# IvanBanny/para-ortho-pca-bo

Measured on AMD Instinct MI355X. Metric: BO iterations/sec (incl. GP refit + EI opt), BBOB f15 d=40, higher is better.
Workload: dtype f64; 1 GPU; configs[1]: PCA_BO on BBOB f15 d=40, budget=450, n_DoE=120, EI, var_threshold=0.95; one run per GPU (run list f15/d40/instances 0..N-1 partitioned by pcabo.sharding), timed steps spread evenly over the 330 BO iterations of the run; num_restarts=10, raw_samples=512, batch_limit=5, maxiter=200, parallelism=run-parallel x1

## Files before the change

### para-ortho-pca-bo_amd/csrc/ctx_layout.h

```cpp
#pragma once
#include <stddef.h>

#define PCABO_BS 64
#define PCABO_SLAB 16
#define PCABO_MAXD 128
#define PCABO_PSTRIDE (2 + 2 * PCABO_MAXD)
#define PCABO_QA_MAX 416
#define PCABO_CNT_DONE 0x3fff
#define PCABO_QFLAG_WORDS 32
#define PCABO_GROUP_CNT_OFFSET 8192
#define PCABO_HYP_INV_LS 0
#define PCABO_HYP_NOISE 1
#define PCABO_HYP_MEAN_C 2
#define PCABO_HYP_ARD_FOLD 3
#define PCABO_HYP_WORDS 4
#define PCABO_OPT_REC_BASE 64
#define PCABO_OPT_REC_STRIDE 8
static_assert(PCABO_QFLAG_WORDS <= PCABO_OPT_REC_BASE, "the values of a call's restarts end in front of the records");
#define PCABO_XQ_TAIL 8
#define EXT_XN 0
#define EXT_YS PCABO_MAXD
#define EXT_HDR_RUNG (PCABO_MAXD + 1)
#define EXT_HDR_INFO (PCABO_MAXD + 2)
#define EXT_HDR 2
#define EXT_INFO_SKIP (-1)
// ... 109 lines not shown
static inline Use xq_ext_rows(const CtxShape& s, int k) { return {0, (size_t)ext_rows_cap(s, k) * k}; }
static inline Use xq_ext_vals(const CtxShape& s, int k) { return {xq_ext_rows(s, k).count, (size_t)ext_rows_cap(s, k)}; }

static inline Use partial_ext_scratch(const CtxShape& s) { return {0, 3 * (size_t)s.NPcap + EXT_SMALL}; }
struct ExtScratch {
  double *ks, *v, *w, *small;
  ExtScratch(double* partial, const CtxShape& s) : ks(partial), v(partial + s.NPcap), w(partial + 2 * (size_t)s.NPcap), small(partial + 3 * (size_t)s.NPcap) {}
};
static inline Use partial_loo(int n) { return {0, 4 * (size_t)n}; }
static inline size_t partial_loo_part(int n, int v) { return (size_t)v * n; }
static inline Use partial_post_records(int q, int NP) { return {0, (size_t)q * (NP / 64) * PCABO_PSTRIDE}; }
static inline Use partial_post_result(int q, int NP) { return {partial_post_records(q, NP).count, 3 * (size_t)q}; }

static inline Use counters_queries(int q) { return {0, (size_t)q}; }
static inline Use counters_group() { return {PCABO_GROUP_CNT_OFFSET, PCABO_QFLAG_WORDS}; }

static inline Use gram_rt(int NP, int ld) { return {0, (size_t)NP * ld}; }

static inline Use mll_partials(int NP, int M) { const size_t nb = NP / PCABO_BS; return {0, (1 + (size_t)M) * (nb * (nb + 1) / 2)}; }
static inline Use mll_result(int NP, int M) { return {mll_partials(NP, M).count, 5 + (size_t)M}; }
static inline Use hmll_result(int M) { return {0, 5 + (size_t)M}; }

static inline int opt_groups(int num_restarts, int batch_limit) { return (num_restarts + batch_limit - 1) / batch_limit; }
static inline Use xq_opt_points(int num_restarts, int kmax) { return {0, (size_t)(num_restarts + 2) * kmax}; }
static inline Use grad_opt_cands(int num_restarts, int kmax) { return {0, (size_t)num_restarts * kmax}; }
static inline Use val_opt_values(int num_restarts) { return {0, (size_t)num_restarts}; }
static inline Use val_opt_records(int ngroups) { return {PCABO_OPT_REC_BASE, (size_t)PCABO_OPT_REC_STRIDE * ngroups}; }
static inline size_t val_opt_record(int gi) { return PCABO_OPT_REC_BASE + (size_t)PCABO_OPT_REC_STRIDE * gi; }
static inline bool opt_fits(const CtxLayout& L, int num_restarts, int ngroups, int kmax) {
  return fits(val_opt_records(ngroups), L.dev[D_VAL]) && fits(xq_opt_points(num_restarts, kmax), xq_queries(L.s));
// ... 2 lines not shown
```

### para-ortho-pca-bo_amd/csrc/host_selftest.cpp

```cpp
#include "../../include/pcabo.h"
#include "host_side.h"
#include "lb_plan.h"
#include "ctx_layout.h"
#include "model_state.h"

#include <atomic>
#include <cmath>
#include <cstdint>
#include <cstdio>
#include <cstdlib>
#include <cstring>
#include <vector>

namespace {

int g_fail = 0;
#define CHECK(c, ...) do { if (!(c)) { std::fprintf(stderr, "FAIL %s:%d: ", __FILE__, __LINE__); std::fprintf(stderr, __VA_ARGS__); std::fprintf(stderr, "\n"); ++g_fail; } } while (0)

struct Lcg {
  uint64_t s;
  explicit Lcg(uint64_t seed) : s(seed * 6364136223846793005ull + 1442695040888963407ull) {}
  double uni() { s = s * 6364136223846793005ull + 1442695040888963407ull; return (double)(s >> 11) * (1.0 / 9007199254740992.0); }
};

// ... 921 lines not shown
             val_opt_record(0) == 64 && val_opt_record(ngroups - 1) + 8 == rec.start + rec.count, "the device optimiser's values and records");
    }
    for (int M : {1, s.KPcap}) {
      const Use part = mll_partials(s.NPcap, M), res = mll_result(s.NPcap, M);
      LCHECK(fits(part, L.dev[D_MLL]) && fits(res, L.dev[D_MLL]) && apart(part, res) && fits(hmll_result(M), L.host[H_MLL]) &&
             hmll_result(M).count == res.count, "the fit's results");
    }
    const Use w = small_wpca(s), x = small_imap_x(s), nb = small_norm_bounds(s);
    const PcaParts pp = pca_parts(s);
    LCHECK(fits(w, small) && fits(x, small) && fits(nb, small) && apart(w, x) && apart(w, nb) && apart(x, nb), "the three tenants of hSmall");
    LCHECK(x.count >= (size_t)max_d && nb.count >= 2 * (size_t)max_d && pca_copy_count(s, max_d, max_d) == w.count && w.count == L.dev[D_PCAOUT].count &&
           pp.data_mean + max_d <= pp.pca_mean && pp.pca_mean + max_d <= pp.evr && pp.evr + max_d <= pp.comps, "the wPCA result block");
    LCHECK(in_pack(max_n, max_d, true, true, true).total == L.dev[D_IN].count && L.dev[D_IN].count == L.host[H_IN].count, "the packed inputs");
    LCHECK(fits(counters_queries(max_q), L.dev[D_COUNTERS]) && fits(counters_group(), L.dev[D_COUNTERS]) &&
           apart(counters_queries(PCABO_QFLAG_WORDS), counters_group()), "the tickets");
    LCHECK(fits(gram_rt(s.NPcap, s.NPcap), L.dev[D_GRAM]), "the transposed root inverse");
#undef LCHECK
  }
}

struct MS {
  int n, n_base, d, k, KP, NP; double ls, s2; int kernel; double rung;
  bool have_wpca, unc; int wn, wd; bool pending, have_gp, zn, rt; int cnt_S; bool dirty; int gcur, vprev_d;
};
void expect_state(const ModelState& s, const MS& e, const char* what) {
  CHECK(s.n == e.n && s.n_base == e.n_base && s.d == e.d && s.k == e.k && s.KP == e.KP && s.NP == e.NP,
        "%s: shape n %d n_base %d d %d k %d KP %d NP %d", what, s.n, s.n_base, s.d, s.k, s.KP, s.NP);
  CHECK(s.lengthscale == e.ls && s.noise == e.s2 && s.kernel == e.kernel && s.rung == e.rung,
        "%s: hyperparameters %g %g %d rung %g", what, s.lengthscale, s.noise, s.kernel, s.rung);
  CHECK(s.have_wpca == e.have_wpca && s.wpca_uncollected == e.unc && s.wpca_n == e.wn && s.wpca_d == e.wd,
// ... 207 lines not shown
```

### para-ortho-pca-bo_amd/csrc/kernels_acq.hip

```cpp
#include "pcabo_internal.h"
#include "acq_math.h"
#include <algorithm>
#include <cstdlib>
#include <mutex>

#define PSTRIDE PCABO_PSTRIDE

#ifdef PCABO_ACQ_TIMING
__device__ unsigned long long g_acq_stamps[16];
#define STAMP(i) do { if (blockIdx.x == gridDim.x / 2 && blockIdx.y == 0 && threadIdx.x == 0) g_acq_stamps[i] = wall_clock64(); } while (0)
#define STAMP_FIN(i) do { if (blockIdx.y == 0 && threadIdx.x == 0) g_acq_stamps[i] = wall_clock64(); } while (0)
extern "C" int pcabo_debug_acq_stamps(unsigned long long* out16) {
  return hipMemcpyFromSymbol(out16, HIP_SYMBOL(g_acq_stamps), sizeof(g_acq_stamps)) == hipSuccess ? 0 : -3;
}
#else
#define STAMP(i)
#define STAMP_FIN(i)
#endif

__device__ inline void st_wt(double* p, double v) {
  __hip_atomic_store(p, v, __ATOMIC_RELAXED, __HIP_MEMORY_SCOPE_AGENT);
}

template <int SLAB>
// ... 1119 lines not shown
  const int tid = threadIdx.x, l = tid & 63, w = tid >> 6;
  const int j = blockIdx.x * 256 + tid, q0 = blockIdx.y * SC_QB;
  double ks[SC_QB];
  score_ks_block(Xq, q_total, n, k, NP, ld, ZnT, bounds4, prm, KS, ks);
  const double aj = j < n ? alpha[j] : 0.0;
#pragma unroll
  for (int q = 0; q < SC_QB; ++q) {
    const double m = wave_sum(aj * ks[q]);
    if (l == 0) s_mu[w][q] = m;
  }
  __syncthreads();
  if (tid < SC_QB && q0 + tid < q_total)
    partial[((size_t)(q0 + tid) * S + blockIdx.x) * PSTRIDE + 1] = ((s_mu[0][tid] + s_mu[1][tid]) + s_mu[2][tid]) + s_mu[3][tid];
}

template <bool STORE_V>
__global__ __launch_bounds__(256) void k_score_gemm(const double* __restrict__ R, const double* __restrict__ KS,
                                                    int q_total, int NP, int ld, int njb, double* __restrict__ partial,
                                                    double* __restrict__ V, size_t zs, size_t vzs) {
  ZRUN(R); ZRUN(KS); ZRUN(partial);
  __shared__ __attribute__((aligned(16))) double s_a[64 * PCABO_TLD];
  __shared__ __attribute__((aligned(16))) double s_b[64 * PCABO_TLD];
  __shared__ double s_red[4][64];
  const int tid = threadIdx.x, w = tid >> 6, l = tid & 63;
  const int I = blockIdx.x, qb = blockIdx.y, S = gridDim.x;
  const double* Rrow = R + (size_t)(I * 64) * ld;
  const double* Krow = KS + (size_t)(qb * 64) * ld;
  double4_t acc[4];
  tile_product_f64<false>(s_a, s_b, I + 1, [&](int J, int r, int c, double& a, double& b) {
    a = Rrow[(size_t)r * ld + J * 64 + c];
    b = (qb * 64 + r < q_total) ? Krow[(size_t)r * ld + J * 64 + c] : 0.0;
  }, acc);
  if (STORE_V) {
    V = zrun(V, vzs, blockIdx.z);
#pragma unroll
    for (int t = 0; t < 4; ++t) {
      const int a = qb * 64 + 16 * t + (l & 15);
#pragma unroll
      for (int r = 0; r < 4; ++r)
        if (a < q_total) V[(size_t)(I * 64 + 16 * w + (l >> 4) + 4 * r) * q_total + a] = acc[t][r];
    }
  }
#pragma unroll
  for (int t = 0; t < 4; ++t) {
    double v = ((acc[t][0] * acc[t][0] + acc[t][1] * acc[t][1]) + acc[t][2] * acc[t][2]) + acc[t][3] * acc[t][3];
    v += __shfl_xor(v, 16, 64);
    v += __shfl_xor(v, 32, 64);
    if (l < 16) s_red[w][16 * t + l] = v;
  }
  __syncthreads();
  if (tid < 64 && qb * 64 + tid < q_total) {
    double* rec = partial + ((size_t)(qb * 64 + tid) * S + I) * PSTRIDE;
    rec[0] = ((s_red[0][tid] + s_red[1][tid]) + s_red[2][tid]) + s_red[3][tid];
    if (I >= njb) rec[1] = 0.0;
  }
}

void launch_score_gemm(hipStream_t st, const GpModel& m, int q, const double* KS, double* partial, size_t zs, int B, double* V,
                       size_t vzs) {
  const dim3 grid(m.NP / 64, (q + 63) / 64, B);
  const int njb = (m.NP + 255) / 256;
  if (V) hipLaunchKernelGGL(k_score_gemm<true>, grid, dim3(256), 0, st, m.R, KS, q, m.NP, m.ld, njb, partial, V, zs, vzs);
  else hipLaunchKernelGGL(k_score_gemm<false>, grid, dim3(256), 0, st, m.R, KS, q, m.NP, m.ld, njb, partial, V, zs, vzs);
}

bool score_gemm_possible(int q) { return q >= 64; }

__global__ __launch_bounds__(256) void k_score_ks_only(const double* __restrict__ Xq, int q_total, int n, int k, int NP, int ld,
                                                       const double* __restrict__ ZnT, const double* __restrict__ bounds4,
                                                       AcqParams prm, double* __restrict__ KS) {
  double ks[SC_QB];
  score_ks_block(Xq, q_total, n, k, NP, ld, ZnT, bounds4, prm, KS, ks);
}

__global__ __launch_bounds__(256) void k_score_mu(const double* __restrict__ KS, int q_total, int n, int ld,
                                                  const double* __restrict__ alpha, double* __restrict__ partial, int S) {
  __shared__ double s_mu[4][SC_QB];
  const int tid = threadIdx.x, l = tid & 63, w = tid >> 6;
  const int j = blockIdx.x * 256 + tid, q0 = blockIdx.y * SC_QB;
  const double aj = j < n ? alpha[j] : 0.0;
#pragma unroll
  for (int q = 0; q < SC_QB; ++q) {
    const double ks = (j < n && q0 + q < q_total) ? KS[(size_t)(q0 + q) * ld + j] : 0.0;
    const double m = wave_sum(aj * ks);
    if (l == 0) s_mu[w][q] = m;
  }
  __syncthreads();
  if (tid < SC_QB && q0 + tid < q_total)
    partial[((size_t)(q0 + tid) * S + blockIdx.x) * PSTRIDE + 1] = ((s_mu[0][tid] + s_mu[1][tid]) + s_mu[2][tid]) + s_mu[3][tid];
}

void launch_score_ks_only(hipStream_t st, const double* Xq, int q, const GpModel& m, AcqParams p, double* KS) {
  const int njb = (m.NP + 255) / 256;
  hipLaunchKernelGGL(k_score_ks_only, dim3(njb, (q + SC_QB - 1) / SC_QB, 1), dim3(256), 0, st, Xq, q, m.n, m.k, m.NP, m.ld, m.ZnT,
                     m.bounds4, p, KS);
}
void launch_score_tail(hipStream_t st, int q, const GpModel& m, AcqParams p, const double* KS, double* partial, double* val) {
  const int S = m.NP / 64, njb = (m.NP + 255) / 256;
  hipLaunchKernelGGL(k_score_mu, dim3(njb, (q + SC_QB - 1) / SC_QB, 1), dim3(256), 0, st, KS, q, m.n, m.ld, m.alpha, partial, S);
  launch_score_gemm(st, m, q, KS, partial);
  p.want_grad = 0;
  hipLaunchKernelGGL(k_acq_combine, dim3((q + 3) / 4, 1, 1), dim3(256), 0, st, partial, q, S, m.k, m.bounds4, m.ystats, p, val,
                     (double*)nullptr, AcqBatch());
}

void launch_score_ks(hipStream_t st, const double* Xq, int q, const GpModel& m, AcqParams p, double* KS, double* partial, AcqBatch ab,
                     int B) {
  const int S = m.NP / 64, njb = (m.NP + 255) / 256;
  hipLaunchKernelGGL(k_score_ks, dim3(njb, (q + SC_QB - 1) / SC_QB, B), dim3(256), 0, st, Xq, q, m.n, m.k, m.NP, m.ld, m.ZnT, m.alpha,
                     m.bounds4, p, KS, partial, S, ab);
}

void launch_score(hipStream_t st, const double* Xq, int q, const GpModel& m, AcqParams p, double* KS, double* partial, double* val,
                  AcqBatch ab, int B) {
  const int S = m.NP / 64;
  launch_score_ks(st, Xq, q, m, p, KS, partial, ab, B);
  launch_score_gemm(st, m, q, KS, partial, ab.zs, B);
  p.want_grad = 0;
// ... 105 lines not shown
```

### para-ortho-pca-bo_amd/csrc/kernels_gp.hip

```cpp
#include "pcabo_internal.h"
#include <mutex>
#include <cstdlib>

#define BS PCABO_BS
#define TLD PCABO_TLD

__global__ __launch_bounds__(256) void k_gram(const double* __restrict__ AT, const double* __restrict__ nrm, int n,
                                              int KP, int ld, double noise, int kernel, double* __restrict__ K,
                                              const int* __restrict__ k_dev, double* __restrict__ K2,
                                              int* __restrict__ info_reset, size_t zs, const double* __restrict__ hyp) {
  const XcdTile xt_ = xcd_tile();
  ZRUNX(AT); ZRUNX(nrm); ZRUNX(K); ZRUNX(k_dev); ZRUNX(K2); ZRUNX(info_reset); ZRUNX(hyp);
  if (hyp) noise = hyp[PCABO_HYP_NOISE];
  const int ti = (int)xt_.x, tj = (int)xt_.y;
  if (info_reset && ti == 0 && tj == 0 && threadIdx.x == 0) *info_reset = 0;
  if (tj > ti) return;
  if (k_dev) KP = (*k_dev + 3) & ~3;
  const int w = threadIdx.x >> 6, l = threadIdx.x & 63;
  const int i0 = ti * BS + 16 * w, j0 = tj * BS;
  double4_t acc[4];
  for (int t = 0; t < 4; ++t) acc[t] = (double4_t){0.0, 0.0, 0.0, 0.0};
  for (int kk = 0; kk < KP; kk += 4) {
    const double* row = AT + (size_t)(kk + (l >> 4)) * ld;
    double a = row[i0 + (l & 15)];
// ... 249 lines not shown
    __syncthreads();
    double4_t x = {0.0, 0.0, 0.0, 0.0};
    for (int kk = 0; kk < BS; kk += 4) {
      double a = s_t[(16 * w + (l & 15)) * TLD + kk + (l >> 4)];
      double b = s_xk[(kk + (l >> 4)) * 16 + (l & 15)];
      x = __builtin_amdgcn_mfma_f64_16x16x4f64(a, b, x, 0, 0, 0);
    }
    for (int r = 0; r < 4; ++r)
      R[(size_t)(I * BS + 16 * w + (l >> 4) + 4 * r) * ld + c0 + (l & 15)] = x[r];
    __threadfence_block();
  }
}

__device__ __forceinline__ void rmatvec_run(const double* __restrict__ R, const double* __restrict__ y, int n, int ld,
                                            double* __restrict__ t) {
  const int w = threadIdx.x >> 6, l = threadIdx.x & 63;
  for (int rr = 0; rr < 4; ++rr) {
    const int i = blockIdx.x * 16 + w * 4 + rr;
    double s = 0.0;
    if (i < n)
      for (int j = l; j <= i; j += 64) s += R[(size_t)i * ld + j] * y[j];
    s = wave_sum(s);
    if (l == 0) t[i] = (i < n) ? s : 0.0;
  }
}
__global__ __launch_bounds__(256) void k_rmatvec(const double* __restrict__ R, const double* __restrict__ y, int n,
                                                 int ld, double* __restrict__ t, size_t zs) {
  ZRUN(R); ZRUN(y); ZRUN(t);
  rmatvec_run(R, y, n, ld, t);
}
__global__ __launch_bounds__(256) void k_rmatvec_gated(const double* __restrict__ R, const double* __restrict__ y, int n, int ld,
                                                       double* __restrict__ t, size_t zs, const int* __restrict__ gate) {
  if (*zrun(gate, zs, blockIdx.z) != 0) return;
  ZRUN(R); ZRUN(y); ZRUN(t);
  rmatvec_run(R, y, n, ld, t);
}

#define RTM_WAVES 16
__device__ __forceinline__ void rtmatvec_run(const double* __restrict__ R, const double* __restrict__ t, int n, int ld,
// ... 19 lines not shown
    out[j] = (j < n) ? s : 0.0;
  }
}
__global__ __launch_bounds__(64 * RTM_WAVES) void k_rtmatvec(const double* __restrict__ R, const double* __restrict__ t,
                                                             int n, int ld, double* __restrict__ out, size_t zs) {
  ZRUN(R); ZRUN(t); ZRUN(out);
  rtmatvec_run(R, t, n, ld, out);
}
__global__ __launch_bounds__(64 * RTM_WAVES) void k_rtmatvec_gated(const double* __restrict__ R, const double* __restrict__ t, int n,
                                                                   int ld, double* __restrict__ out, size_t zs,
                                                                   const int* __restrict__ gate) {
  if (*zrun(gate, zs, blockIdx.z) != 0) return;
  ZRUN(R); ZRUN(t); ZRUN(out);
  rtmatvec_run(R, t, n, ld, out);
}

void launch_gram(hipStream_t s, const double* AT, const double* nrm, int n, int NP, int KP, int ld, double noise,
                 int kernel, double* K, const int* k_dev, double* K2, int* info_reset, ZB zb) {
  int nb = NP / BS;
  hipLaunchKernelGGL(k_gram, dim3(nb, nb, zb.B), dim3(256), 0, s, AT, nrm, n, KP, ld, noise, kernel, K, k_dev, K2, info_reset,
                     zb.zs, zb.hyp);
}
void launch_add_jitter(hipStream_t s, double* K, int n, int ld, double jitter) {
  hipLaunchKernelGGL(k_add_jitter, dim3((n + 255) / 256), dim3(256), 0, s, K, n, ld, jitter);
}
bool chol_step_form(int NP, ZB zb) { return zb.B * (NP / BS) <= 256; }
int launch_cholesky(hipStream_t s, double* L, int NP, int ld, int* info, double* diag_scratch, ZB zb, double* R_folded) {
  const int nblk = NP / BS;
  if (chol_step_form(NP, zb)) return launch_chol_steps(s, L, NP, ld, info, diag_scratch, zb, R_folded);
  if (R_folded) return -1;
// ... 36 lines not shown
      }
    }
  }
  return 0;
}
void launch_trinv(hipStream_t s, const double* L, int NP, int ld, double* R, ZB zb) {
  const int nblk = NP / BS;
  launch_trinv_diag_w(s, L, nblk, ld, R, zb);
  hipLaunchKernelGGL(k_trinv_cols, dim3(NP / 16, 1, zb.B), dim3(256), 0, s, L, nblk, ld, R, zb.zs);
}
void launch_alpha(hipStream_t s, const double* R, const double* ys, int n, int NP, int ld, double* tmp, double* alpha,
                  ZB zb) {
  hipLaunchKernelGGL(k_rmatvec, dim3(NP / 16, 1, zb.B), dim3(256), 0, s, R, ys, n, ld, tmp, zb.zs);
  hipLaunchKernelGGL(k_rtmatvec, dim3(NP / 64, 1, zb.B), dim3(64 * RTM_WAVES), 0, s, R, tmp, n, ld, alpha, zb.zs);
}
void launch_alpha_gated(hipStream_t s, const double* R, const double* ys, int n, int NP, int ld, double* tmp, double* alpha, ZB zb,
                        const int* gate) {
  hipLaunchKernelGGL(k_rmatvec_gated, dim3(NP / 16, 1, zb.B), dim3(256), 0, s, R, ys, n, ld, tmp, zb.zs, gate);
  hipLaunchKernelGGL(k_rtmatvec_gated, dim3(NP / 64, 1, zb.B), dim3(64 * RTM_WAVES), 0, s, R, tmp, n, ld, alpha, zb.zs, gate);
}
```

### para-ortho-pca-bo_amd/csrc/kernels_gpw.hip

```cpp
#include "pcabo_internal.h"
#include <mutex>

#define BS PCABO_BS
#ifdef PCABO_ACQ_TIMING
__device__ unsigned long long g_panel_stamps[16];
extern "C" int pcabo_debug_panel_stamps(unsigned long long* out16) {
  return hipMemcpyFromSymbol(out16, HIP_SYMBOL(g_panel_stamps), sizeof(g_panel_stamps)) == hipSuccess ? 0 : -3;
}
#define PSTAMP(i) do { if (blockIdx.x == 0 && blockIdx.z == 0 && threadIdx.x == 0) g_panel_stamps[i] = wall_clock64(); } while (0)
#else
#define PSTAMP(i)
#endif
#define WLD 65

__device__ inline double lane_get(double v, int lane) {
  return __hiloint2double(__builtin_amdgcn_readlane(__double2hiint(v), lane),
                          __builtin_amdgcn_readlane(__double2loint(v), lane));
}


#define PANEL_LDS_SYNC() asm volatile("s_waitcnt lgkmcnt(0)" ::: "memory")
template <int JB, bool LOWER>
__device__ inline void tiles_colblock_to_lds(const double4_t (&acc)[4][4], double* s_t, int l) {
#pragma unroll
// ... 534 lines not shown
  InvChunk<0, 0, 0>::run(x, lb, s_lt, s_rd, xm);
  double* dst = R + (size_t)(b * BS) * ld + b * BS;
#pragma unroll
  for (int r = 0; r < BS; ++r) dst[(size_t)r * ld + c] = (r >= c) ? x[r] : 0.0;
}


void launch_chol_panel(hipStream_t s, double* L, int p, int nblocks, int ld, int* info, double* diag_scratch, ZB zb) {
  hipLaunchKernelGGL(k_chol_panel_m, dim3(nblocks, 1, zb.B), dim3(128), 0, s, L, p, ld, info, diag_scratch, zb.zs);
}
__global__ __launch_bounds__(256) void k_trinv_rowblock(const double* L, int I, int ld, double* R) {
  __shared__ __attribute__((aligned(16))) double s_t[BS * SLD];
  __shared__ __attribute__((aligned(16))) double s_xk[BS * 16];
  trinv_rowblock_chunk(L, R, I, 16 * blockIdx.x, ld, s_t, s_xk);
}
void launch_trinv_drain(hipStream_t s, const double* L, int NP, int ld, double* R) {
  const int nblk = NP / BS;
  if (nblk >= 2) hipLaunchKernelGGL(k_trinv_rowblock, dim3(4 * (nblk - 1)), dim3(256), 0, s, L, nblk - 1, ld, R);
}
int launch_chol_steps(hipStream_t s, double* L, int NP, int ld, int* info, double* diag_scratch, ZB zb, double* R) {
  static std::mutex attr_mu;
  static bool attr_done[64] = {false};
  int dev = 0;
  if (hipGetDevice(&dev) != hipSuccess || dev < 0 || dev >= 64) return -1;
  {
    std::lock_guard<std::mutex> lk(attr_mu);
    if (!attr_done[dev]) {
      if (hipFuncSetAttribute((const void*)k_chol_step, hipFuncAttributeMaxDynamicSharedMemorySize, (int)CHOL_STEP_LDS) != hipSuccess) return -1;
      attr_done[dev] = true;
    }
  }
  const int nblk = NP / BS;
  for (int J = 0; J < nblk; ++J) {
// ... 9 lines not shown
```

### para-ortho-pca-bo_amd/csrc/pcabo_api.hip

```cpp
#include "../../include/pcabo.h"
#include "pcabo_internal.h"
#include "lbfgsb.h"
#include "host_side.h"
#include "model_state.h"

#include <algorithm>
#include <atomic>
#include <chrono>
#include <thread>
#include <condition_variable>
#include <functional>
#include <mutex>
#include <cstdlib>
#include <cmath>
#include <cstdio>
#include <cstring>
#include <new>
#include <optional>
#include <vector>
#include <dirent.h>
#include <fcntl.h>
#include <signal.h>
#include <stdint.h>
#include <cerrno>
// ... 355 lines not shown
  int n, k, KP; const int* k_dev;
  double inv_ls, noise, mean_c; int kernel;
  ZB zb;
  hipEvent_t ev[2];
  bool reset_tickets;
  const double* ard_ls = nullptr;
  hipEvent_t ev_zn = nullptr;
};
template <class Phase>
static int enqueue_factor(pcabo_ctx* ctx, hipStream_t s, int n, int NP, ZB zb, Phase&& phase) {
  if (const int rc = phase(2)) return rc;
  const bool fold = !ctx->in_batch && ctx->opt_hidden_tail && zb.zs == 0 && zb.B == 1 && chol_step_form(NP, zb);
  if (launch_cholesky(s, ctx->dL, NP, ctx->ld, ctx->dInfo, ctx->dDiag, zb, fold ? ctx->dR : nullptr) != 0)
    return set_err(ctx, PCABO_ERR_HIP, "the Cholesky launches could not be set up (device or kernel attribute)%s", "");
  if (const int rc = phase(3)) return rc;
  if (fold) launch_trinv_drain(s, ctx->dL, NP, ctx->ld, ctx->dR);
  else launch_trinv(s, ctx->dL, NP, ctx->ld, ctx->dR, zb);
  launch_alpha(s, ctx->dR, ctx->dYs, n, NP, ctx->ld, ctx->dTmp, ctx->dAlpha, zb);
  if (const int rc = phase(4)) return rc;
  if (zb.zs) HIPCHK(hipMemcpy2DAsync((void*)&ctx->hm->chol_info, zb.hzs, ctx->dInfo, zb.zs, sizeof(int), zb.B, hipMemcpyDeviceToHost, s));
  else HIPCHK(hipMemcpyAsync((void*)&ctx->hm->chol_info, ctx->dInfo, sizeof(int), hipMemcpyDeviceToHost, s));
  return PCABO_OK;
}
template <class Phase>
static int enqueue_rows_dh(pcabo_ctx* ctx, hipStream_t s, const RowsDH& a, Phase&& phase) {
  const int NP = round_up(a.n, PCABO_BS);
  if (a.reset_tickets) {
    if (a.zb.zs) HIPCHK(hipMemset2DAsync(ctx->dCounters, a.zb.zs, 0, ticket_bytes(ctx), a.zb.B, s));
    else HIPCHK(hipMemsetAsync(ctx->dCounters, 0, ticket_bytes(ctx), s));
  }
// ... 469 lines not shown
    launch_acq(s, qa, xdev, nq, gp_model(ctx), p, ctx->dPartial, ctx->dCounters, ctx->dVal, ctx->dGrad, small ? ctx->hVal : nullptr,
               small ? ctx->hGrad : nullptr, small ? ctx->hm : nullptr, seq);
  }
  if (!small) {
    HIPCHK(hipMemcpyAsync(ctx->hVal, ctx->dVal, (size_t)nq * sizeof(double), hipMemcpyDeviceToHost, s));
    if (p.want_grad) HIPCHK(hipMemcpyAsync(ctx->hGrad, ctx->dGrad, (size_t)nq * k * sizeof(double), hipMemcpyDeviceToHost, s));
    HIPCHK(wait_stream(s));
    HIPCHK(hipGetLastError());
    return PCABO_OK;
  }
  return acq_published(ctx, wait_flags(ctx->hm, 0, nq, seq, deadline_in(20), &s));
}

static int score_tail(pcabo_ctx* ctx, int nq, AcqParams& p) {
  hipStream_t s = ctx->stream;
  launch_score_tail(s, nq, gp_model(ctx), p, ctx->dKS, ctx->dPartial, ctx->dVal);
  HIPCHK(hipMemcpyAsync(ctx->hVal, ctx->dVal, (size_t)nq * sizeof(double), hipMemcpyDeviceToHost, s));
  HIPCHK(wait_stream(s));
  HIPCHK(hipGetLastError());
  return PCABO_OK;
}

struct GroupLaunches {
  int g0[8], gn[8], ng = 0;
  void add(int q0, int n) { g0[ng] = q0; gn[ng] = n; ++ng; }
};
static int eval_staged_groups(pcabo_ctx* ctx, const GroupLaunches& t, AcqParams& p) {
  hipStream_t s = ctx->stream;
  const unsigned long long seq = ++ctx->seq;
  const int *g0 = t.g0, *gn = t.gn, ng = t.ng;
  QueryArgs tab;
  unsigned* ent = reinterpret_cast<unsigned*>(tab.x);
// ... 2019 lines not shown
```

### para-ortho-pca-bo_amd/csrc/pcabo_internal.h

```cpp
#pragma once
#include <hip/hip_runtime.h>
#include <stdint.h>
#include <type_traits>
#include "ctx_layout.h"

#define PCABO_TLD 66
#define PCABO_INLAUNCH_MAXQ 32
static_assert(PCABO_INLAUNCH_MAXQ == PCABO_QFLAG_WORDS, "one sequence word of the host mirror per query finished inside a launch");

typedef double double4_t __attribute__((ext_vector_type(4)));
struct QueryArgs { double x[PCABO_QA_MAX]; };
struct alignas(16) MailPair { double v; unsigned long long tag; };
static inline __host__ __device__ unsigned long long mail_mix(unsigned long long vbits) {
  const unsigned int lo = (unsigned int)vbits, hi = (unsigned int)(vbits >> 32);
  return (unsigned long long)((lo ^ hi ^ (hi >> 11)) & 0xFFFFFFu);
}
#define PCABO_MAIL_PAIRS (1 + PCABO_QA_MAX + PCABO_INLAUNCH_MAXQ + 1)
#define PCABO_SERVER_TIMEOUT_TICKS 200000000ull

#ifdef __HIPCC__
__device__ inline double fast_rcp(double x) {
  double r = __builtin_amdgcn_rcp(x);
  r = fma(fma(-x, r, 1.0), r, r);
  r = fma(fma(-x, r, 1.0), r, r);
// ... 98 lines not shown
__device__ inline double row_sum16(double v) {
  v += dpp_get<0xB1, 0xf>(v);
  v += dpp_get<0x4E, 0xf>(v);
  v += dpp_get<0x141, 0xf>(v);
  v += dpp_get<0x140, 0xf>(v);
  return v;
}
__device__ inline double wave_sum(double v) {
  v = row_sum16(v);
  v += dpp_get<0x142, 0xa>(v);
  v += dpp_get<0x143, 0xc>(v);
  return __hiloint2double(__builtin_amdgcn_readlane(__double2hiint(v), 63),
                          __builtin_amdgcn_readlane(__double2loint(v), 63));
}

template <bool KMAJOR, typename Elem>
__device__ __forceinline__ void tile_product_f64(double* s_a, double* s_b, int steps, Elem elem, double4_t (&acc)[4]) {
  const int tid = threadIdx.x, w = tid >> 6, l = tid & 63;
  double pa[16], pb[16];
  auto fetch = [&](int J) {
#pragma unroll
    for (int u = 0; u < 16; ++u) {
      const int idx = tid + 256 * u;
      elem(J, idx >> 6, idx & 63, pa[u], pb[u]);
    }
  };
  auto put = [&]() {
#pragma unroll
    for (int u = 0; u < 16; ++u) {
      const int idx = tid + 256 * u, r = idx >> 6, c = idx & 63;
      s_a[r * PCABO_TLD + c] = pa[u];
      s_b[r * PCABO_TLD + c] = pb[u];
    }
  };
#pragma unroll
  for (int t = 0; t < 4; ++t) acc[t] = (double4_t){0.0, 0.0, 0.0, 0.0};
  fetch(0);
  for (int J = 0; J < steps; ++J) {
    __syncthreads();
    put();
    if (J + 1 < steps) fetch(J + 1);
    __syncthreads();
    for (int kk = 0; kk < 64; kk += 4) {
      const double a = KMAJOR ? s_a[(kk + (l >> 4)) * PCABO_TLD + 16 * w + (l & 15)]
                              : s_a[(16 * w + (l & 15)) * PCABO_TLD + kk + (l >> 4)];
#pragma unroll
      for (int t = 0; t < 4; ++t) {
        const double b = KMAJOR ? s_b[(kk + (l >> 4)) * PCABO_TLD + 16 * t + (l & 15)]
                                : s_b[(16 * t + (l & 15)) * PCABO_TLD + kk + (l >> 4)];
        acc[t] = __builtin_amdgcn_mfma_f64_16x16x4f64(a, b, acc[t], 0, 0, 0);
      }
    }
  }
}

template <int T>
__device__ inline double lane_xor(double v) {
  if (T == 0) return dpp_get<0xB1, 0xf>(v);
  if (T == 1) return dpp_get<0x4E, 0xf>(v);
  if (T == 2) return dpp_get<0x141, 0xf>(dpp_get<0x1B, 0xf>(v));
  return dpp_get<0x128, 0xf>(v);
}
// ... 82 lines not shown
                    const double* comps, const int* k_dev, int n, int d, double* Z, ZB zb = ZB());
void launch_zstats(hipStream_t s, const double* Z, const double* y, int n, int k, const double* user_norm_bounds,
                   double* bounds4 , double* zn_mean, double* ystats,
                   double* ys, HostMirror* hm, const int* k_dev = nullptr, ZB zb = ZB(),
                   double mean_c = 0.0,
                   const double* ard_ls = nullptr);
void launch_znorm(hipStream_t s, const double* Z, int n, int k, int NP, int KP, int ld, const double* bounds4,
                  const double* zn_mean, double inv_ls, double* ZnT, double* AT, double* nrm,
                  const int* k_dev = nullptr, ZB zb = ZB());
void launch_gram(hipStream_t s, const double* AT, const double* nrm, int n, int NP, int KP, int ld, double noise,
                 int kernel, double* K, const int* k_dev = nullptr, double* K2 = nullptr, int* info_reset = nullptr,
                 ZB zb = ZB());
void launch_add_jitter(hipStream_t s, double* K, int n, int ld, double jitter);
int launch_cholesky(hipStream_t s, double* L, int NP, int ld, int* info, double* diag_scratch, ZB zb = ZB(), double* R_folded = nullptr);
bool chol_step_form(int NP, ZB zb);
void launch_trinv_drain(hipStream_t s, const double* L, int NP, int ld, double* R);
void launch_trinv(hipStream_t s, const double* L, int NP, int ld, double* R, ZB zb = ZB());
void launch_chol_panel(hipStream_t s, double* L, int p, int nblocks, int ld, int* info, double* diag_scratch, ZB zb = ZB());
int launch_chol_steps(hipStream_t s, double* L, int NP, int ld, int* info, double* diag_scratch , ZB zb = ZB(),
                      double* R = nullptr);
void launch_trinv_diag_w(hipStream_t s, const double* L, int nblk, int ld, double* R, ZB zb = ZB());
void launch_alpha(hipStream_t s, const double* R, const double* ys, int n, int NP, int ld, double* tmp, double* alpha,
                  ZB zb = ZB());
void launch_alpha_gated(hipStream_t s, const double* R, const double* ys, int n, int NP, int ld, double* tmp, double* alpha, ZB zb,
                        const int* gate);
void launch_mll_grad(hipStream_t s, bool ard, const double* R, const double* AT, const double* nrm, const double* alpha,
                     const double* L, const double* ys, int n, int NP, int KP, int ld, double* partial, double* out,
                     const int* k_dev = nullptr, ZB zb = ZB());
void launch_acq(hipStream_t s, const QueryArgs* qa, const double* Xq, int q, const GpModel& m, AcqParams p, double* partial,
                unsigned int* counters, double* val, double* grad, double* host_val, double* host_grad, HostMirror* hm,
                unsigned long long seq,
                MailPair* dev_mail = nullptr, MailPair* part_pairs = nullptr,
                AcqBatch ab = AcqBatch(), int B = 1, int table_entries = 0);
#define PCABO_GROUP_Q 5
bool acq_group_possible(int NP, int k);
int launch_acq_group(hipStream_t st, const QueryArgs* tab, int entries, const double* Xq, const GpModel& m, AcqParams p,
                     double* partial, unsigned int* counters, double* val, double* grad, double* host_val, double* host_grad,
                     HostMirror* hm, unsigned long long seq, AcqBatch ab);
// ... 9 lines not shown
                      double* KS, double* partial, double* post, double* V, double* cov, AcqBatch ab = AcqBatch(),
                      size_t vzs = 0, int B = 1);
void launch_post_chol_prep(hipStream_t st, const double* cov, int q, const double* ystats, double jitter, double* F, int* info,
                           size_t zs = 0, size_t vzs = 0, size_t szs = 0, int B = 1);
void launch_post_sample(hipStream_t st, const double* F, int q, const double* base, int S, const double* mean ,
                        double* out, size_t zs = 0, size_t szs = 0, int B = 1);
void launch_loo(hipStream_t st, const double* R, const double* alpha, const double* ys, const double* ystats, int n, int ld,
                double* out, size_t zs = 0, int B = 1);
struct GpArrays { const double* zn_mean; double *L, *R, *ZnT, *AT, *nrm, *ys; };
void launch_ext_ks(hipStream_t st, const double* X, int xi, const double* Y, int yi, const GpModel& m, double inv_ls, int kernel,
                   const ExtScratch& e, AcqBatch ab = AcqBatch(), int B = 1);
void launch_ext_append(hipStream_t st, const GpModel& m, const ExtScratch& e, int idx, int believer, double s2, double inv_ls,
                       const GpArrays& a, AcqBatch ab = AcqBatch(), int B = 1);
void launch_ext_truncate(hipStream_t st, const ExtScratch& e, int n0, int k, int NP, int ld, const GpArrays& a,
                         AcqBatch ab = AcqBatch(), int B = 1);
void launch_score_tail(hipStream_t st, int q, const GpModel& m, AcqParams p, const double* KS, double* partial, double* val);
bool acq_server_possible(int q, int n, int k, int NP);
int acq_slabs(int NP);
void launch_inverse_map(hipStream_t s, const double* z, const double* comps, const double* data_mean,
                        const double* pca_mean, int k, int d, double* x, const int* k_dev = nullptr, ZB zb = ZB(),
                        double* host_x = nullptr, HostMirror* hm = nullptr, unsigned long long seq = 0);
void launch_rt_build(hipStream_t s, const double* R, int n, int NP, int ld, double* RT, ZB zb = ZB());
bool lbfgsb_device_possible(int NP, int kmax, int batch_limit);
int launch_lbfgsb_group(hipStream_t st, const unsigned* table, int entries, int mode, int num_restarts, int maxiter, const GpModel& m,
                        const double* Xq, const double* RT, const double* bestf, const int* k_dev, double inv_ls,
                        int maximize, int acq, int kernel, double* out_x, double* out_v, size_t zs,
                        const double* hyp = nullptr,
                        int batch_limit = PCABO_GROUP_Q);
```

Baseline: 420.1 BO iterations/s.

## Fuse score tail kernels with ticketed finish and merge alpha solve into trinv drain

The scoring tail's three launches (mu, GEMM column norms, combine) become one kernel. Its blocks do either the GEMM slab or the mu block, and the last block per query group, found through an atomic ticket counter, runs the EI finish and writes values straight to host memory, so the separate device-to-host copy goes away. In the GP refit, the R*y matvec rides along in the trinv drain launch, and a tail kernel finishes the last rows, does the transposed matvec and publishes chol_info to the host mirror. This cuts launches and a memcpy per call, at the cost of a narrower GEMM tile, counter-based cross-block sync and extra correctness risk.

```diff
diff --git a/para-ortho-pca-bo_amd/csrc/ctx_layout.h b/para-ortho-pca-bo_amd/csrc/ctx_layout.h
--- a/para-ortho-pca-bo_amd/csrc/ctx_layout.h
+++ b/para-ortho-pca-bo_amd/csrc/ctx_layout.h
@@ -9,6 +9,7 @@
 #define PCABO_CNT_DONE 0x3fff
 #define PCABO_QFLAG_WORDS 32
 #define PCABO_GROUP_CNT_OFFSET 8192
+#define PCABO_SCORE_CNT_OFFSET 12288
 #define PCABO_HYP_INV_LS 0
 #define PCABO_HYP_NOISE 1
 #define PCABO_HYP_MEAN_C 2
@@ -148,6 +149,7 @@
 
 static inline Use counters_queries(int q) { return {0, (size_t)q}; }
 static inline Use counters_group() { return {PCABO_GROUP_CNT_OFFSET, PCABO_QFLAG_WORDS}; }
+static inline Use counters_score(int q) { return {PCABO_SCORE_CNT_OFFSET, ((size_t)q + 15) / 16}; }
 
 static inline Use gram_rt(int NP, int ld) { return {0, (size_t)NP * ld}; }
 
diff --git a/para-ortho-pca-bo_amd/csrc/host_selftest.cpp b/para-ortho-pca-bo_amd/csrc/host_selftest.cpp
--- a/para-ortho-pca-bo_amd/csrc/host_selftest.cpp
+++ b/para-ortho-pca-bo_amd/csrc/host_selftest.cpp
@@ -959,6 +959,8 @@
     LCHECK(in_pack(max_n, max_d, true, true, true).total == L.dev[D_IN].count && L.dev[D_IN].count == L.host[H_IN].count, "the packed inputs");
     LCHECK(fits(counters_queries(max_q), L.dev[D_COUNTERS]) && fits(counters_group(), L.dev[D_COUNTERS]) &&
            apart(counters_queries(PCABO_QFLAG_WORDS), counters_group()), "the tickets");
+    LCHECK(fits(counters_score(max_q), L.dev[D_COUNTERS]) && apart(counters_score(max_q), counters_group()) &&
+           apart(counters_score(max_q), counters_queries(PCABO_QFLAG_WORDS)), "the scoring's tickets");
     LCHECK(fits(gram_rt(s.NPcap, s.NPcap), L.dev[D_GRAM]), "the transposed root inverse");
 #undef LCHECK
   }
diff --git a/para-ortho-pca-bo_amd/csrc/kernels_acq.hip b/para-ortho-pca-bo_amd/csrc/kernels_acq.hip
--- a/para-ortho-pca-bo_amd/csrc/kernels_acq.hip
+++ b/para-ortho-pca-bo_amd/csrc/kernels_acq.hip
@@ -1157,6 +1157,17 @@
     partial[((size_t)(q0 + tid) * S + blockIdx.x) * PSTRIDE + 1] = ((s_mu[0][tid] + s_mu[1][tid]) + s_mu[2][tid]) + s_mu[3][tid];
 }
 
+template <int NT>
+__device__ __forceinline__ void score_colnorms(const double4_t (&acc)[NT], double* red, int l) {
+#pragma unroll
+  for (int t = 0; t < NT; ++t) {
+    double v = __builtin_fma(acc[t][3], acc[t][3], __builtin_fma(acc[t][2], acc[t][2], __builtin_fma(acc[t][0], acc[t][0], acc[t][1] * acc[t][1])));
+    v += __shfl_xor(v, 16, 64);
+    v += __shfl_xor(v, 32, 64);
+    if (l < 16) red[16 * t + l] = v;
+  }
+}
+
 template <bool STORE_V>
 __global__ __launch_bounds__(256) void k_score_gemm(const double* __restrict__ R, const double* __restrict__ KS,
                                                     int q_total, int NP, int ld, int njb, double* __restrict__ partial,
@@ -1184,13 +1195,7 @@
         if (a < q_total) V[(size_t)(I * 64 + 16 * w + (l >> 4) + 4 * r) * q_total + a] = acc[t][r];
     }
   }
-#pragma unroll
-  for (int t = 0; t < 4; ++t) {
-    double v = ((acc[t][0] * acc[t][0] + acc[t][1] * acc[t][1]) + acc[t][2] * acc[t][2]) + acc[t][3] * acc[t][3];
-    v += __shfl_xor(v, 16, 64);
-    v += __shfl_xor(v, 32, 64);
-    if (l < 16) s_red[w][16 * t + l] = v;
-  }
+  score_colnorms(acc, s_red[w], l);
   __syncthreads();
   if (tid < 64 && qb * 64 + tid < q_total) {
     double* rec = partial + ((size_t)(qb * 64 + tid) * S + I) * PSTRIDE;
@@ -1216,11 +1221,10 @@
   score_ks_block(Xq, q_total, n, k, NP, ld, ZnT, bounds4, prm, KS, ks);
 }
 
-__global__ __launch_bounds__(256) void k_score_mu(const double* __restrict__ KS, int q_total, int n, int ld,
-                                                  const double* __restrict__ alpha, double* __restrict__ partial, int S) {
-  __shared__ double s_mu[4][SC_QB];
+__device__ __forceinline__ void score_mu_block(const double* __restrict__ KS, int q_total, int n, int ld, const double* __restrict__ alpha,
+                                               double* partial, int S, int jb, int q0, double (*s_mu)[SC_QB]) {
   const int tid = threadIdx.x, l = tid & 63, w = tid >> 6;
-  const int j = blockIdx.x * 256 + tid, q0 = blockIdx.y * SC_QB;
+  const int j = jb * 256 + tid;
   const double aj = j < n ? alpha[j] : 0.0;
 #pragma unroll
   for (int q = 0; q < SC_QB; ++q) {
@@ -1230,7 +1234,65 @@
   }
   __syncthreads();
   if (tid < SC_QB && q0 + tid < q_total)
-    partial[((size_t)(q0 + tid) * S + blockIdx.x) * PSTRIDE + 1] = ((s_mu[0][tid] + s_mu[1][tid]) + s_mu[2][tid]) + s_mu[3][tid];
+    st_wt(&partial[((size_t)(q0 + tid) * S + jb) * PSTRIDE + 1], ((s_mu[0][tid] + s_mu[1][tid]) + s_mu[2][tid]) + s_mu[3][tid]);
+}
+
+__global__ __launch_bounds__(256) void k_score_fused(const double* __restrict__ R, const double* __restrict__ KS,
+                                                     const double* __restrict__ alpha, int q_total, int n, int NP, int ld, int k,
+                                                     const double* __restrict__ bounds4, const double* __restrict__ ystats,
+                                                     AcqParams p, double* partial, unsigned int* tickets, double* val,
+                                                     double* host_val) {
+  __shared__ __attribute__((aligned(16))) double s_a[64 * PCABO_TLD];
+  __shared__ __attribute__((aligned(16))) double s_b[SC_QB * PCABO_TLD];
+  __shared__ double s_red[4][SC_QB];
+  __shared__ int s_last;
+  const int tid = threadIdx.x, w = tid >> 6, l = tid & 63;
+  const int S = NP / 64, njb = (NP + 255) / 256, Q16 = (q_total + SC_QB - 1) / SC_QB;
+  const int b = blockIdx.x;
+  int qb;
+  if (b < S * Q16) {
+    const int I = S - 1 - b / Q16;
+    qb = b % Q16;
+    const int q0 = qb * SC_QB;
+    const double* Rrow = R + (size_t)(I * 64) * ld;
+    const double* Krow = KS + (size_t)q0 * ld;
+    double4_t acc[1];
+    tile_product_f64<false>(s_a, s_b, I + 1, [&](int J, int r, int c, double& a, double& bv) {
+      a = Rrow[(size_t)r * ld + J * 64 + c];
+      bv = (r < SC_QB && q0 + r < q_total) ? Krow[(size_t)r * ld + J * 64 + c] : 0.0;
+    }, acc);
+    score_colnorms(acc, s_red[w], l);
+    __syncthreads();
+    if (tid < SC_QB && q0 + tid < q_total) {
+      double* rec = partial + ((size_t)(q0 + tid) * S + I) * PSTRIDE;
+      st_wt(rec, ((s_red[0][tid] + s_red[1][tid]) + s_red[2][tid]) + s_red[3][tid]);
+      if (I >= njb) st_wt(rec + 1, 0.0);
+    }
+  } else {
+    const int b2 = b - S * Q16;
+    qb = b2 / njb;
+    score_mu_block(KS, q_total, n, ld, alpha, partial, S, b2 % njb, qb * SC_QB, s_red);
+  }
+  asm volatile("s_waitcnt vmcnt(0)" ::: "memory");
+  __syncthreads();
+  if (tid == 0) {
+    const unsigned int t = __hip_atomic_fetch_add(&tickets[qb], 1u, __ATOMIC_RELAXED, __HIP_MEMORY_SCOPE_AGENT);
+    const int last = t == (unsigned int)(S + njb - 1);
+    if (last) {
+      __builtin_amdgcn_fence(__ATOMIC_ACQUIRE, "agent");
+      asm volatile("s_waitcnt vmcnt(0)" ::: "memory");
+      __hip_atomic_store(&tickets[qb], 0u, __ATOMIC_RELAXED, __HIP_MEMORY_SCOPE_AGENT);
+    }
+    s_last = last;
+  }
+  __syncthreads();
+  if (!s_last) return;
+  p.want_grad = 0;
+  for (int u = 0; u < 4; ++u) {
+    const int q = qb * SC_QB + 4 * w + u;
+    if (q < q_total)
+      acq_finish_query(partial + (size_t)q * S * PSTRIDE, S, k, q, bounds4, ystats, p, val, nullptr, host_val, nullptr, l);
+  }
 }
 
 void launch_score_ks_only(hipStream_t st, const double* Xq, int q, const GpModel& m, AcqParams p, double* KS) {
@@ -1238,13 +1300,11 @@
   hipLaunchKernelGGL(k_score_ks_only, dim3(njb, (q + SC_QB - 1) / SC_QB, 1), dim3(256), 0, st, Xq, q, m.n, m.k, m.NP, m.ld, m.ZnT,
                      m.bounds4, p, KS);
 }
-void launch_score_tail(hipStream_t st, int q, const GpModel& m, AcqParams p, const double* KS, double* partial, double* val) {
-  const int S = m.NP / 64, njb = (m.NP + 255) / 256;
-  hipLaunchKernelGGL(k_score_mu, dim3(njb, (q + SC_QB - 1) / SC_QB, 1), dim3(256), 0, st, KS, q, m.n, m.ld, m.alpha, partial, S);
-  launch_score_gemm(st, m, q, KS, partial);
-  p.want_grad = 0;
-  hipLaunchKernelGGL(k_acq_combine, dim3((q + 3) / 4, 1, 1), dim3(256), 0, st, partial, q, S, m.k, m.bounds4, m.ystats, p, val,
-                     (double*)nullptr, AcqBatch());
+void launch_score_tail(hipStream_t st, int q, const GpModel& m, AcqParams p, const double* KS, double* partial, unsigned int* tickets,
+                       double* val, double* host_val) {
+  const int S = m.NP / 64, njb = (m.NP + 255) / 256, Q16 = (q + SC_QB - 1) / SC_QB;
+  hipLaunchKernelGGL(k_score_fused, dim3((S + njb) * Q16), dim3(256), 0, st, m.R, KS, m.alpha, q, m.n, m.NP, m.ld, m.k, m.bounds4,
+                     m.ystats, p, partial, tickets, val, host_val);
 }
 
 void launch_score_ks(hipStream_t st, const double* Xq, int q, const GpModel& m, AcqParams p, double* KS, double* partial, AcqBatch ab,
diff --git a/para-ortho-pca-bo_amd/csrc/kernels_gp.hip b/para-ortho-pca-bo_amd/csrc/kernels_gp.hip
--- a/para-ortho-pca-bo_amd/csrc/kernels_gp.hip
+++ b/para-ortho-pca-bo_amd/csrc/kernels_gp.hip
@@ -287,15 +287,7 @@
 
 __device__ __forceinline__ void rmatvec_run(const double* __restrict__ R, const double* __restrict__ y, int n, int ld,
                                             double* __restrict__ t) {
-  const int w = threadIdx.x >> 6, l = threadIdx.x & 63;
-  for (int rr = 0; rr < 4; ++rr) {
-    const int i = blockIdx.x * 16 + w * 4 + rr;
-    double s = 0.0;
-    if (i < n)
-      for (int j = l; j <= i; j += 64) s += R[(size_t)i * ld + j] * y[j];
-    s = wave_sum(s);
-    if (l == 0) t[i] = (i < n) ? s : 0.0;
-  }
+  rmatvec_rows16(R, y, n, ld, t, blockIdx.x * 16);
 }
 __global__ __launch_bounds__(256) void k_rmatvec(const double* __restrict__ R, const double* __restrict__ y, int n,
                                                  int ld, double* __restrict__ t, size_t zs) {
@@ -345,6 +337,19 @@
   ZRUN(R); ZRUN(t); ZRUN(out);
   rtmatvec_run(R, t, n, ld, out);
 }
+__global__ __launch_bounds__(64 * RTM_WAVES) void k_rtmatvec_tail(const double* __restrict__ R, const double* __restrict__ y, int n,
+                                                                  int NP, int ld, double* t, double* __restrict__ out,
+                                                                  const int* __restrict__ info, HostMirror* hm) {
+  const int w = threadIdx.x >> 6, l = threadIdx.x & 63;
+  for (int rr = 0; rr < 4; ++rr) {
+    const int i = NP - 64 + 4 * w + rr;
+    const double s = rmatvec_row(R, y, n, ld, i, l);
+    if (l == 0) t[i] = s;
+  }
+  __syncthreads();
+  rtmatvec_run(R, t, n, ld, out);
+  if (blockIdx.x == 0 && threadIdx.x == 0) __hip_atomic_store(&hm->chol_info, *info, __ATOMIC_RELAXED, __HIP_MEMORY_SCOPE_SYSTEM);
+}
 
 void launch_gram(hipStream_t s, const double* AT, const double* nrm, int n, int NP, int KP, int ld, double noise,
                  int kernel, double* K, const int* k_dev, double* K2, int* info_reset, ZB zb) {
@@ -411,6 +416,10 @@
   hipLaunchKernelGGL(k_rmatvec, dim3(NP / 16, 1, zb.B), dim3(256), 0, s, R, ys, n, ld, tmp, zb.zs);
   hipLaunchKernelGGL(k_rtmatvec, dim3(NP / 64, 1, zb.B), dim3(64 * RTM_WAVES), 0, s, R, tmp, n, ld, alpha, zb.zs);
 }
+void launch_alpha_tail(hipStream_t s, const double* R, const double* ys, int n, int NP, int ld, double* tmp, double* alpha,
+                       const int* info, HostMirror* hm) {
+  hipLaunchKernelGGL(k_rtmatvec_tail, dim3(NP / 64), dim3(64 * RTM_WAVES), 0, s, R, ys, n, NP, ld, tmp, alpha, info, hm);
+}
 void launch_alpha_gated(hipStream_t s, const double* R, const double* ys, int n, int NP, int ld, double* tmp, double* alpha, ZB zb,
                         const int* gate) {
   hipLaunchKernelGGL(k_rmatvec_gated, dim3(NP / 16, 1, zb.B), dim3(256), 0, s, R, ys, n, ld, tmp, zb.zs, gate);
diff --git a/para-ortho-pca-bo_amd/csrc/kernels_gpw.hip b/para-ortho-pca-bo_amd/csrc/kernels_gpw.hip
--- a/para-ortho-pca-bo_amd/csrc/kernels_gpw.hip
+++ b/para-ortho-pca-bo_amd/csrc/kernels_gpw.hip
@@ -572,9 +572,19 @@
   __shared__ __attribute__((aligned(16))) double s_xk[BS * 16];
   trinv_rowblock_chunk(L, R, I, 16 * blockIdx.x, ld, s_t, s_xk);
 }
-void launch_trinv_drain(hipStream_t s, const double* L, int NP, int ld, double* R) {
+__global__ __launch_bounds__(256) void k_trinv_drain_t(const double* L, int I, int ld, double* R, const double* __restrict__ ys,
+                                                       int n, double* __restrict__ t) {
+  __shared__ __attribute__((aligned(16))) double s_t[BS * SLD];
+  __shared__ __attribute__((aligned(16))) double s_xk[BS * 16];
+  const int nchunk = 4 * I;
+  if ((int)blockIdx.x < nchunk) trinv_rowblock_chunk(L, R, I, 16 * blockIdx.x, ld, s_t, s_xk);
+  else rmatvec_rows16(R, ys, n, ld, t, 16 * ((int)blockIdx.x - nchunk));
+}
+void launch_trinv_drain(hipStream_t s, const double* L, int NP, int ld, double* R, const double* ys, int n, double* t) {
   const int nblk = NP / BS;
-  if (nblk >= 2) hipLaunchKernelGGL(k_trinv_rowblock, dim3(4 * (nblk - 1)), dim3(256), 0, s, L, nblk - 1, ld, R);
+  if (nblk < 2) return;
+  if (ys) hipLaunchKernelGGL(k_trinv_drain_t, dim3(8 * (nblk - 1)), dim3(256), 0, s, L, nblk - 1, ld, R, ys, n, t);
+  else hipLaunchKernelGGL(k_trinv_rowblock, dim3(4 * (nblk - 1)), dim3(256), 0, s, L, nblk - 1, ld, R);
 }
 int launch_chol_steps(hipStream_t s, double* L, int NP, int ld, int* info, double* diag_scratch, ZB zb, double* R) {
   static std::mutex attr_mu;
diff --git a/para-ortho-pca-bo_amd/csrc/pcabo_api.hip b/para-ortho-pca-bo_amd/csrc/pcabo_api.hip
--- a/para-ortho-pca-bo_amd/csrc/pcabo_api.hip
+++ b/para-ortho-pca-bo_amd/csrc/pcabo_api.hip
@@ -393,6 +393,11 @@
   if (launch_cholesky(s, ctx->dL, NP, ctx->ld, ctx->dInfo, ctx->dDiag, zb, fold ? ctx->dR : nullptr) != 0)
     return set_err(ctx, PCABO_ERR_HIP, "the Cholesky launches could not be set up (device or kernel attribute)%s", "");
   if (const int rc = phase(3)) return rc;
+  if (fold && !ctx->prof) {
+    launch_trinv_drain(s, ctx->dL, NP, ctx->ld, ctx->dR, ctx->dYs, n, ctx->dTmp);
+    launch_alpha_tail(s, ctx->dR, ctx->dYs, n, NP, ctx->ld, ctx->dTmp, ctx->dAlpha, ctx->dInfo, ctx->hm);
+    return phase(4);
+  }
   if (fold) launch_trinv_drain(s, ctx->dL, NP, ctx->ld, ctx->dR);
   else launch_trinv(s, ctx->dL, NP, ctx->ld, ctx->dR, zb);
   launch_alpha(s, ctx->dR, ctx->dYs, n, NP, ctx->ld, ctx->dTmp, ctx->dAlpha, zb);
@@ -892,8 +897,7 @@
 
 static int score_tail(pcabo_ctx* ctx, int nq, AcqParams& p) {
   hipStream_t s = ctx->stream;
-  launch_score_tail(s, nq, gp_model(ctx), p, ctx->dKS, ctx->dPartial, ctx->dVal);
-  HIPCHK(hipMemcpyAsync(ctx->hVal, ctx->dVal, (size_t)nq * sizeof(double), hipMemcpyDeviceToHost, s));
+  launch_score_tail(s, nq, gp_model(ctx), p, ctx->dKS, ctx->dPartial, ctx->dCounters + counters_score(nq).start, ctx->dVal, ctx->hVal);
   HIPCHK(wait_stream(s));
   HIPCHK(hipGetLastError());
   return PCABO_OK;
diff --git a/para-ortho-pca-bo_amd/csrc/pcabo_internal.h b/para-ortho-pca-bo_amd/csrc/pcabo_internal.h
--- a/para-ortho-pca-bo_amd/csrc/pcabo_internal.h
+++ b/para-ortho-pca-bo_amd/csrc/pcabo_internal.h
@@ -136,15 +136,34 @@
                           __builtin_amdgcn_readlane(__double2loint(v), 63));
 }
 
-template <bool KMAJOR, typename Elem>
-__device__ __forceinline__ void tile_product_f64(double* s_a, double* s_b, int steps, Elem elem, double4_t (&acc)[4]) {
+__device__ __forceinline__ double rmatvec_row(const double* __restrict__ R, const double* __restrict__ y, int n, int ld, int i, int l) {
+  double s = 0.0;
+  if (i < n)
+    for (int j = l; j <= i; j += 64) s = __builtin_fma(R[(size_t)i * ld + j], y[j], s);
+  s = wave_sum(s);
+  return (i < n) ? s : 0.0;
+}
+__device__ __forceinline__ void rmatvec_rows16(const double* __restrict__ R, const double* __restrict__ y, int n, int ld,
+                                               double* __restrict__ t, int row0) {
+  const int w = threadIdx.x >> 6, l = threadIdx.x & 63;
+  for (int rr = 0; rr < 4; ++rr) {
+    const int i = row0 + w * 4 + rr;
+    const double s = rmatvec_row(R, y, n, ld, i, l);
+    if (l == 0) t[i] = s;
+  }
+}
+
+template <bool KMAJOR, int NT = 4, typename Elem>
+__device__ __forceinline__ void tile_product_f64(double* s_a, double* s_b, int steps, Elem elem, double4_t (&acc)[NT]) {
+  static_assert(NT >= 1 && NT <= 4 && (NT == 4 || !KMAJOR), "a narrower second tile is cut by rows: row-major tiles");
   const int tid = threadIdx.x, w = tid >> 6, l = tid & 63;
-  double pa[16], pb[16];
+  double pa[16], pb[4 * NT];
   auto fetch = [&](int J) {
 #pragma unroll
     for (int u = 0; u < 16; ++u) {
       const int idx = tid + 256 * u;
-      elem(J, idx >> 6, idx & 63, pa[u], pb[u]);
+      double unused;
+      elem(J, idx >> 6, idx & 63, pa[u], u < 4 * NT ? pb[u < 4 * NT ? u : 0] : unused);
     }
   };
   auto put = [&]() {
@@ -152,11 +171,11 @@
     for (int u = 0; u < 16; ++u) {
       const int idx = tid + 256 * u, r = idx >> 6, c = idx & 63;
       s_a[r * PCABO_TLD + c] = pa[u];
-      s_b[r * PCABO_TLD + c] = pb[u];
+      if (u < 4 * NT) s_b[r * PCABO_TLD + c] = pb[u < 4 * NT ? u : 0];
     }
   };
 #pragma unroll
-  for (int t = 0; t < 4; ++t) acc[t] = (double4_t){0.0, 0.0, 0.0, 0.0};
+  for (int t = 0; t < NT; ++t) acc[t] = (double4_t){0.0, 0.0, 0.0, 0.0};
   fetch(0);
   for (int J = 0; J < steps; ++J) {
     __syncthreads();
@@ -167,7 +186,7 @@
       const double a = KMAJOR ? s_a[(kk + (l >> 4)) * PCABO_TLD + 16 * w + (l & 15)]
                               : s_a[(16 * w + (l & 15)) * PCABO_TLD + kk + (l >> 4)];
 #pragma unroll
-      for (int t = 0; t < 4; ++t) {
+      for (int t = 0; t < NT; ++t) {
         const double b = KMAJOR ? s_b[(kk + (l >> 4)) * PCABO_TLD + 16 * t + (l & 15)]
                                 : s_b[(16 * t + (l & 15)) * PCABO_TLD + kk + (l >> 4)];
         acc[t] = __builtin_amdgcn_mfma_f64_16x16x4f64(a, b, acc[t], 0, 0, 0);
@@ -280,7 +299,8 @@
 void launch_add_jitter(hipStream_t s, double* K, int n, int ld, double jitter);
 int launch_cholesky(hipStream_t s, double* L, int NP, int ld, int* info, double* diag_scratch, ZB zb = ZB(), double* R_folded = nullptr);
 bool chol_step_form(int NP, ZB zb);
-void launch_trinv_drain(hipStream_t s, const double* L, int NP, int ld, double* R);
+void launch_trinv_drain(hipStream_t s, const double* L, int NP, int ld, double* R, const double* ys = nullptr, int n = 0,
+                        double* t = nullptr);
 void launch_trinv(hipStream_t s, const double* L, int NP, int ld, double* R, ZB zb = ZB());
 void launch_chol_panel(hipStream_t s, double* L, int p, int nblocks, int ld, int* info, double* diag_scratch, ZB zb = ZB());
 int launch_chol_steps(hipStream_t s, double* L, int NP, int ld, int* info, double* diag_scratch , ZB zb = ZB(),
@@ -288,6 +308,8 @@
 void launch_trinv_diag_w(hipStream_t s, const double* L, int nblk, int ld, double* R, ZB zb = ZB());
 void launch_alpha(hipStream_t s, const double* R, const double* ys, int n, int NP, int ld, double* tmp, double* alpha,
                   ZB zb = ZB());
+void launch_alpha_tail(hipStream_t s, const double* R, const double* ys, int n, int NP, int ld, double* tmp, double* alpha,
+                       const int* info, HostMirror* hm);
 void launch_alpha_gated(hipStream_t s, const double* R, const double* ys, int n, int NP, int ld, double* tmp, double* alpha, ZB zb,
                         const int* gate);
 void launch_mll_grad(hipStream_t s, bool ard, const double* R, const double* AT, const double* nrm, const double* alpha,
@@ -327,7 +349,8 @@
                        const GpArrays& a, AcqBatch ab = AcqBatch(), int B = 1);
 void launch_ext_truncate(hipStream_t st, const ExtScratch& e, int n0, int k, int NP, int ld, const GpArrays& a,
                          AcqBatch ab = AcqBatch(), int B = 1);
-void launch_score_tail(hipStream_t st, int q, const GpModel& m, AcqParams p, const double* KS, double* partial, double* val);
+void launch_score_tail(hipStream_t st, int q, const GpModel& m, AcqParams p, const double* KS, double* partial, unsigned int* tickets,
+                       double* val, double* host_val);
 bool acq_server_possible(int q, int n, int k, int NP);
 int acq_slabs(int NP);
 void launch_inverse_map(hipStream_t s, const double* z, const double* comps, const double* data_mean,
```

Measured after the change: 428.2 BO iterations/s (median of 2 runs). Within noise of the previous version (+1.9%).
